# weikaolun/horovod-distributed-example

Measured on AMD Instinct MI355X. Metric: images/sec (whole node) + scaling efficiency, ResNet-50 bf16 at 1/2/4/8 MI355X, higher is better.
Workload: dtype bf16; 1 GPU; model=ResNet-50, global_batch=2048, per_gpu_batch=2048, image=224, parallelism=dp1, optimizer=mivod FusedSGD via DistributedOptimizer, compression=none, transport=local, hip_graph=False

## Files before the change

### csrc/kernels/mv_gemm.hip

```cpp
#include "mv_mfma.h"
#include "mv_gemm.h"

#include <cstdlib>

namespace mv {
namespace gemm {

constexpr int BK = 64;
constexpr int KC = BK / 8;

template <int BM, int BN, int WM, int WN, bool STATS>
__global__ __launch_bounds__(WM * WN * 64) void gemm_nt_kernel(
    const __bf16* __restrict__ A, const __bf16* __restrict__ B, __bf16* __restrict__ C,
    int64_t M, int N, int K, int ntn, const float* __restrict__ shift,
    float* __restrict__ partial) {
  constexpr int NT = WM * WN * 64;
  constexpr int A_CH = BM * KC / NT;
  constexpr int B_CH = BN * KC / NT;
  constexpr int WTM = BM / WM, WTN = BN / WN;
  constexpr int TM = WTM / 16, TN = WTN / 16;
  constexpr int STAGE = (BM + BN) * BK;
  static_assert(BM * KC % NT == 0 && BN * KC % NT == 0, "tile / thread mismatch");
  static_assert(WTM % 16 == 0 && WTN % 16 == 0, "wave tile");
  __shared__ __attribute__((aligned(16))) __bf16 smem[2 * STAGE];

  const int tid = threadIdx.x, lane = tid & 63, wid = tid >> 6;
  const int wm = wid / WN, wn = wid % WN;
  const int t = xcd_remap(blockIdx.x, gridDim.x);
  const int mt = t / ntn, nt = t - mt * ntn;
  const int64_t m0 = (int64_t)mt * BM;
  const int n0 = nt * BN;

  u32x4 ra[A_CH], rb[B_CH];
  auto gload = [&](int k0) {
#pragma unroll
    for (int i = 0; i < A_CH; ++i) {
      const int q = tid + i * NT, row = q / KC, ch = q % KC;
      int64_t gm = m0 + row;
      gm = gm < M ? gm : M - 1;
      ra[i] = *reinterpret_cast<const u32x4*>(A + gm * K + k0 + ch * 8);
    }
#pragma unroll
    for (int i = 0; i < B_CH; ++i) {
      const int q = tid + i * NT, row = q / KC, ch = q % KC;
      rb[i] = *reinterpret_cast<const u32x4*>(B + (int64_t)(n0 + row) * K + k0 + ch * 8);
    }
  };
  auto sstore = [&](int buf) {
    __bf16* As = smem + buf * STAGE;
    __bf16* Bs = As + BM * BK;
#pragma unroll
    for (int i = 0; i < A_CH; ++i) {
      const int q = tid + i * NT, row = q / KC, ch = q % KC;
      *reinterpret_cast<u32x4*>(As + swz64(row, ch)) = ra[i];
    }
#pragma unroll
    for (int i = 0; i < B_CH; ++i) {
      const int q = tid + i * NT, row = q / KC, ch = q % KC;
      *reinterpret_cast<u32x4*>(Bs + swz64(row, ch)) = rb[i];
    }
  };

  f32x4v acc[TN][TM];
#pragma unroll
  for (int a = 0; a < TN; ++a)
#pragma unroll
    for (int b = 0; b < TM; ++b) acc[a][b] = f32x4v{0.f, 0.f, 0.f, 0.f};

  const int KT = K / BK;
  gload(0);
  sstore(0);
  __syncthreads();
  for (int kt = 0; kt < KT; ++kt) {
    if (kt + 1 < KT) gload((kt + 1) * BK);
    const __bf16* As = smem + (kt & 1) * STAGE;
    const __bf16* Bs = As + BM * BK;
#pragma unroll
    for (int kk = 0; kk < BK / 32; ++kk) {
      const int ch = kk * 4 + (lane >> 4);
      bf16x8 wf[TN], af[TM];
#pragma unroll
      for (int a = 0; a < TN; ++a)
        wf[a] = *reinterpret_cast<const bf16x8*>(Bs + swz64(wn * WTN + a * 16 + (lane & 15), ch));
#pragma unroll
      for (int b = 0; b < TM; ++b)
        af[b] = *reinterpret_cast<const bf16x8*>(As + swz64(wm * WTM + b * 16 + (lane & 15), ch));
#pragma unroll
      for (int a = 0; a < TN; ++a)
#pragma unroll
        for (int b = 0; b < TM; ++b) acc[a][b] = mfma(wf[a], af[b], acc[a][b]);
    }
    if (kt + 1 < KT) sstore((kt + 1) & 1);
    __syncthreads();
  }

  const int g = lane >> 4, rl = lane & 15;
  float s1[TN][4], s2[TN][4];
#pragma unroll
  for (int a = 0; a < TN; ++a) {
    const int col = n0 + wn * WTN + a * 16 + 4 * g;
    float sh[4] = {0.f, 0.f, 0.f, 0.f};
    if (STATS && shift) {
#pragma unroll
      for (int r = 0; r < 4; ++r) sh[r] = shift[col + r];
    }
#pragma unroll
    for (int r = 0; r < 4; ++r) { s1[a][r] = 0.f; s2[a][r] = 0.f; }
#pragma unroll
    for (int b = 0; b < TM; ++b) {
      const int64_t row = m0 + wm * WTM + b * 16 + rl;
      if (row < M) {
        const f32x4v v = acc[a][b];
        u32x2 o = {cvt_pk_bf16(v[0], v[1]), cvt_pk_bf16(v[2], v[3])};
        *reinterpret_cast<u32x2*>(C + row * N + col) = o;
        if (STATS) {
#pragma unroll
          for (int r = 0; r < 4; ++r) {
            const float d = round_bf16(v[r]) - sh[r];
            s1[a][r] += d;
            s2[a][r] += d * d;
          }
        }
      }
    }
  }
  if (!STATS) return;
#pragma unroll
  for (int a = 0; a < TN; ++a)
#pragma unroll
    for (int r = 0; r < 4; ++r) {
#pragma unroll
      for (int o = 1; o < 16; o <<= 1) {
        s1[a][r] += __shfl_xor(s1[a][r], o, kWave);
        s2[a][r] += __shfl_xor(s2[a][r], o, kWave);
      }
    }
  float* red = reinterpret_cast<float*>(smem);
  if (rl == 0) {
#pragma unroll
    for (int a = 0; a < TN; ++a)
#pragma unroll
      for (int r = 0; r < 4; ++r) {
        const int c = wn * WTN + a * 16 + 4 * g + r;
        red[(0 * WM + wm) * BN + c] = s1[a][r];
        red[(1 * WM + wm) * BN + c] = s2[a][r];
      }
  }
  __syncthreads();
  for (int v = tid; v < 2 * BN; v += NT) {
    const int k = v / BN, c = v - k * BN;
    float s = 0.f;
#pragma unroll
    for (int w = 0; w < WM; ++w) s += red[(k * WM + w) * BN + c];
    partial[((int64_t)mt * 2 + k) * N + n0 + c] = s;
  }
}

struct BwdEpi {
  const __bf16* dy2;
  const uint8_t* mask;
  const __bf16* x;
  const float* mean;
  int ds, H, W;
  const float* sc;
  const float* bi;
  uint8_t* mo;
  const __bf16* a2;
  const float* badd;
  const float* rsc;
  const float* rbi;
  const __bf16* b2;
};

template <int NC>
__device__ __forceinline__ void ld_raw(const __bf16* p, uint32_t (&r)[NC / 2]) {
  if constexpr (NC == 4) {
    const u32x2 w = *reinterpret_cast<const u32x2*>(p);
    r[0] = w[0];
    r[1] = w[1];
  } else {
#pragma unroll
    for (int h = 0; h < NC / 8; ++h) {
      const u32x4 w = *reinterpret_cast<const u32x4*>(p + 8 * h);
#pragma unroll
      for (int j = 0; j < 4; ++j) r[4 * h + j] = w[j];
    }
  }
}

__device__ __forceinline__ float bf_lo(uint32_t w) { return __uint_as_float(w << 16); }
__device__ __forceinline__ float bf_hi(uint32_t w) { return __uint_as_float(w & 0xffff0000u); }

__device__ __forceinline__ int sw64(int row) {
  return (row & 2) | ((((row >> 2) ^ (row >> 4)) & 1) << 2);
}

__device__ __attribute__((aligned(16))) __bf16 g_zero_row[64];
__device__ __attribute__((aligned(16))) __bf16 g_store_scratch[512 * 16];
__device__ __attribute__((aligned(16))) uint8_t g_mask_scratch[512 * 4];

template <int K, int BN, int EPI>
constexpr int stream_wm() {
  if ((EPI == 4 || EPI == 6) && BN == 64) return K == 640 ? 4 : 2;
  return ((EPI == 2 || EPI == 3 || EPI == 5) && (BN == 256 || (K == 256 && BN == 128))) ||
                 ((EPI == 0 || EPI == 1 || EPI == 8) && K == 512)
             ? 2
             : 1;
}

template <int K, int BN, int EPI>
constexpr int stream_wn() {
  return (K == 256 && BN == 128 && (EPI == 2 || EPI == 3 || EPI == 5)) ||
                 ((EPI == 4 || EPI == 6) && BN == 64)
             ? 2
             : 4;
}
template <int K, int BN, int EPI>
constexpr int stream_nt() { return 64 * stream_wn<K, BN, EPI>() * stream_wm<K, BN, EPI>(); }

template <int K, int BN, int EPI, int BM = 64, int K1 = K>
__global__ __launch_bounds__((stream_nt<K, BN, EPI>())) void gemm_stream_kernel(
    const __bf16* __restrict__ A, const __bf16* __restrict__ B, __bf16* __restrict__ C,
    int64_t M, int N, int ntn, int64_t ntm, const float* __restrict__ shift,
    float* __restrict__ partial, BwdEpi be) {
  constexpr int WN = stream_wn<K, BN, EPI>();
  constexpr int NT = stream_nt<K, BN, EPI>();
  constexpr int WM = NT / (64 * WN);
  constexpr int KCH = K / 8;
  constexpr int A_CH = BM * KCH / NT;
  constexpr int W_CH = BN * KCH / NT;
  static_assert(A_CH * NT == BM * KCH && W_CH * NT == BN * KCH, "staging split");
  constexpr int WTN = BN / WN;
  constexpr int WTM = BM / WM;
  constexpr int TN = WTN / 16, TM = WTM / 16;
  constexpr int NC = 4 * TN;
  constexpr bool DUAL = EPI == 7;
  constexpr bool PF = (EPI == 2 || EPI == 3 || EPI == 5) && (BM == 32 || BN == 256);
  __shared__ __attribute__((aligned(16))) __bf16 smem[(BN + BM) * K * (DUAL ? 2 : 1)];
  __bf16* Ws = smem;
  __bf16* As = smem + BN * K;
  __bf16* Ws2 = smem + (BN + BM) * K;
  __bf16* As2 = Ws2 + BN * K;
  constexpr bool SW16 = K % 128 == 0 && K != 128;
  constexpr bool SW64 = K == 64;
  constexpr int LNC = NC == 4 ? 2 : (NC == 8 ? 3 : 4);
  auto swa = [](int row, int ch) {
    return row * K + ((ch ^ (SW16 ? (row & 15) : SW64 ? sw64(row) : (row & 7))) << 3);
  };
  auto sww = [](int row, int ch) {
    return row * K + ((ch ^ (SW16 ? ((row & 3) | (((row >> LNC) & 3) << 2))
                             : SW64 ? sw64(row) : (row & 7))) << 3);
  };

  const int tid = threadIdx.x, lane = tid & 63, wn = (tid >> 6) % WN;
  const int wm = (tid >> 6) / WN;
  const int g = lane >> 4, rl = lane & 15;
  const int t = xcd_remap(blockIdx.x, gridDim.x);
  const int nt = t % ntn;
  const int64_t stream = t / ntn, nstreams = gridDim.x / ntn;
  const int n0 = nt * BN;
  const int cbase = n0 + wn * WTN + NC * g;

#pragma unroll
  for (int i = 0; i < W_CH; ++i) {
    const int q = tid + i * NT, row = q / KCH, ch = q % KCH;
    *reinterpret_cast<u32x4*>(Ws + sww(row, ch)) =
        *reinterpret_cast<const u32x4*>(B + (int64_t)(n0 + row) * K + ch * 8);
    if constexpr (DUAL)
      *reinterpret_cast<u32x4*>(Ws2 + sww(row, ch)) =
          *reinterpret_cast<const u32x4*>(be.b2 + (int64_t)(n0 + row) * K + ch * 8);
  }
  u32x4 ra[A_CH], ra2[DUAL ? A_CH : 1];
  auto gload = [&](u32x4 (&ra)[A_CH], int64_t mt) {
    const int64_t m0 = mt * BM;
#pragma unroll
    for (int i = 0; i < A_CH; ++i) {
      const int q = tid + i * NT, row = q / KCH, ch = q % KCH;
      int64_t gm = m0 + row;
      gm = gm < M ? gm : M - 1;
      if constexpr (K1 == K) {
        ra[i] = *reinterpret_cast<const u32x4*>(A + gm * K + ch * 8);
        if constexpr (DUAL) ra2[i] = *reinterpret_cast<const u32x4*>(be.a2 + gm * K + ch * 8);
      } else {
        const __bf16* p = ch < K1 / 8 ? A + gm * K1 + ch * 8
                                      : be.a2 + gm * (K - K1) + (ch - K1 / 8) * 8;
        ra[i] = *reinterpret_cast<const u32x4*>(p);
      }
    }
  };
  float sh[NC], s1[NC], s2[NC];
  constexpr bool APPLY = EPI == 3 || EPI == 5 || EPI == 7;
  constexpr bool RAFF = EPI == 5 || EPI == 7;
  constexpr bool BADD = EPI == 4 || EPI == 6;
  float apl_sc[EPI >= 3 ? NC : 1], apl_bi[EPI >= 3 ? NC : 1], add[BADD ? NC : 1];
  float res_sc[RAFF ? NC : 1], res_bi[RAFF ? NC : 1];
  if constexpr (RAFF) {
#pragma unroll
    for (int j = 0; j < NC; ++j) {
      res_sc[j] = be.rsc[cbase + j];
      res_bi[j] = be.rbi[cbase + j];
    }
  }
  if constexpr (EPI == 4) {
#pragma unroll
    for (int j = 0; j < NC; ++j) {
      apl_sc[j] = be.sc[cbase + j];
      apl_bi[j] = be.bi[cbase + j];
    }
  }
  if constexpr (BADD) {
#pragma unroll
    for (int j = 0; j < NC; ++j) add[j] = be.badd[cbase + j];
  }
  if constexpr (APPLY) {
    static_assert(NC == 8 || NC == 16, "EPI 3 writes whole mask bytes");
#pragma unroll
    for (int j = 0; j < NC; ++j) {
      apl_sc[j] = be.sc[cbase + j];
      apl_bi[j] = be.bi[cbase + j];
    }
  }
#pragma unroll
  for (int j = 0; j < NC; ++j) {
    sh[j] = 0.f;
    if ((EPI == 1 || EPI == 8) && shift) sh[j] = shift[cbase + j];
    if (EPI == 2 || EPI == 4) sh[j] = be.mean[cbase + j];
    s1[j] = 0.f;
    s2[j] = 0.f;
  }
  struct Epi {
    uint32_t e2[EPI == 2 || APPLY ? TM : 1][NC / 2], ex[EPI == 2 || EPI == 4 ? TM : 1][NC / 2];
    uint32_t em[EPI == 2 ? TM : 1];
  };
  auto load_epi = [&](Epi& E, int64_t mt) {
    auto& e2 = E.e2;
    auto& ex = E.ex;
    auto& em = E.em;
    if constexpr (APPLY && !DUAL) {
#pragma unroll
      for (int b = 0; b < TM; ++b) {
        int64_t row = mt * BM + wm * WTM + b * 16 + rl;
        row = row < M ? row : M - 1;
        ld_raw<NC>(be.dy2 + row * N + cbase, e2[b]);
      }
    }
    if constexpr (EPI == 4) {
#pragma unroll
      for (int b = 0; b < TM; ++b) {
        int64_t row = mt * BM + wm * WTM + b * 16 + rl;
        row = row < M ? row : M - 1;
        ld_raw<NC>(be.x + row * N + cbase, ex[b]);
      }
    }
    if constexpr (EPI == 2) {
#pragma unroll
      for (int b = 0; b < TM; ++b) {
        int64_t row = mt * BM + wm * WTM + b * 16 + rl;
        row = row < M ? row : M - 1;
        int64_t r2 = row;
        bool has = be.dy2 != nullptr;
        if (be.ds > 1) {
          const uint32_t m = (uint32_t)row, hw = (uint32_t)(be.H * be.W);
          const uint32_t n = m / hw, rem = m - n * hw;
          const uint32_t h = rem / (uint32_t)be.W, w = rem - h * (uint32_t)be.W;
          const uint32_t hs = ((uint32_t)be.H + be.ds - 1) / be.ds;
          const uint32_t ws = ((uint32_t)be.W + be.ds - 1) / be.ds;
          has = has && h % be.ds == 0 && w % be.ds == 0;
          r2 = ((int64_t)n * hs + h / be.ds) * ws + w / be.ds;
        }
        ld_raw<NC>(has ? be.dy2 + r2 * N + cbase : g_zero_row, e2[b]);
        ld_raw<NC>(be.x ? be.x + row * N + cbase : g_zero_row, ex[b]);
        const uint8_t* mp = be.mask + row * (N / 8) + cbase / 8;
        if constexpr (NC == 4) em[b] = (uint32_t)mp[0] >> (cbase & 7);
        else if constexpr (NC == 8) em[b] = mp[0];
        else em[b] = *reinterpret_cast<const uint16_t*>(mp);
      }
    }
  };
  auto run_tile = [&](int64_t mt, Epi& E, Epi* En, u32x4 (&ra)[A_CH]) {
    auto& e2 = E.e2;
    auto& ex = E.ex;
    auto& em = E.em;
    (void)e2; (void)ex; (void)em;
    __syncthreads();
#pragma unroll
    for (int i = 0; i < A_CH; ++i) {
      const int q = tid + i * NT, row = q / KCH, ch = q % KCH;
      *reinterpret_cast<u32x4*>(As + swa(row, ch)) = ra[i];
      if constexpr (DUAL) *reinterpret_cast<u32x4*>(As2 + swa(row, ch)) = ra2[i];
    }
    __syncthreads();
    gload(ra, mt + nstreams < ntm ? mt + nstreams : mt);
    if constexpr (PF) {
      __builtin_amdgcn_sched_barrier(0);
      load_epi(*En, mt + nstreams < ntm ? mt + nstreams : mt);
      __builtin_amdgcn_sched_barrier(0);
    }
    f32x4v acc[TN][TM];
#pragma unroll
    for (int a = 0; a < TN; ++a)
#pragma unroll
      for (int b = 0; b < TM; ++b) acc[a][b] = f32x4v{0.f, 0.f, 0.f, 0.f};
    if constexpr (DUAL) {
      f32x4v acc2[TN][TM];
#pragma unroll
      for (int a = 0; a < TN; ++a)
#pragma unroll
        for (int b = 0; b < TM; ++b) acc2[a][b] = f32x4v{0.f, 0.f, 0.f, 0.f};
#pragma unroll
      for (int kk = 0; kk < K / 32; ++kk) {
        const int ch = kk * 4 + g;
        bf16x8 wf[TN], af[TM];
#pragma unroll
        for (int a = 0; a < TN; ++a)
          wf[a] = *reinterpret_cast<const bf16x8*>(
              Ws2 + sww(wn * WTN + NC * (rl >> 2) + 4 * a + (rl & 3), ch));
#pragma unroll
        for (int b = 0; b < TM; ++b)
          af[b] = *reinterpret_cast<const bf16x8*>(As2 + swa(wm * WTM + b * 16 + rl, ch));
#pragma unroll
        for (int a = 0; a < TN; ++a)
#pragma unroll
          for (int b = 0; b < TM; ++b) acc2[a][b] = mfma(wf[a], af[b], acc2[a][b]);
      }
#pragma unroll
      for (int b = 0; b < TM; ++b)
#pragma unroll
        for (int a = 0; a < TN; ++a) {
          e2[b][2 * a] = cvt_pk_bf16(acc2[a][b][0], acc2[a][b][1]);
          e2[b][2 * a + 1] = cvt_pk_bf16(acc2[a][b][2], acc2[a][b][3]);
        }
    }
#pragma unroll
    for (int kk = 0; kk < K / 32; ++kk) {
      const int ch = kk * 4 + g;
      bf16x8 wf[TN], af[TM];
#pragma unroll
      for (int a = 0; a < TN; ++a)
        wf[a] = *reinterpret_cast<const bf16x8*>(
            Ws + sww(wn * WTN + NC * (rl >> 2) + 4 * a + (rl & 3), ch));
#pragma unroll
      for (int b = 0; b < TM; ++b)
        af[b] = *reinterpret_cast<const bf16x8*>(As + swa(wm * WTM + b * 16 + rl, ch));
#pragma unroll
      for (int a = 0; a < TN; ++a)
#pragma unroll
        for (int b = 0; b < TM; ++b) acc[a][b] = mfma(wf[a], af[b], acc[a][b]);
    }
    const int64_t m0 = mt * BM;
#pragma unroll
    for (int b = 0; b < TM; ++b) {
      const int64_t row = m0 + wm * WTM + b * 16 + rl;
      const bool live = row < M;
      uint32_t pk[2 * TN];
#pragma unroll
      for (int a = 0; a < TN; ++a) {
        if constexpr (BADD) {
#pragma unroll
          for (int r = 0; r < 4; ++r) acc[a][b][r] += add[4 * a + r];
        }
        if constexpr (WM >= 2) {
          pk[2 * a] = cvt_pk_bf16_cc(acc[a][b][0], acc[a][b][1]);
          pk[2 * a + 1] = cvt_pk_bf16_cc(acc[a][b][2], acc[a][b][3]);
        } else {
          pk[2 * a] = cvt_pk_bf16(acc[a][b][0], acc[a][b][1]);
          pk[2 * a + 1] = cvt_pk_bf16(acc[a][b][2], acc[a][b][3]);
        }
      }
      float v[NC];
#pragma unroll
      for (int j = 0; j < NC / 2; ++j) {
        v[2 * j] = __uint_as_float(pk[j] << 16);
        v[2 * j + 1] = __uint_as_float(pk[j] & 0xffff0000u);
      }
      if (EPI == 1 || EPI == 8) {
#pragma unroll
        for (int j = 0; j < NC; ++j) {
          const float d = live ? v[j] - sh[j] : 0.f;
          s1[j] += d;
          s2[j] = __builtin_fmaf(d, d, s2[j]);
        }
      }
      if constexpr (EPI == 2) {
#pragma unroll
        for (int j = 0; j < NC / 2; ++j) {
          v[2 * j] += bf_lo(e2[b][j]);
          v[2 * j + 1] += bf_hi(e2[b][j]);
        }
        const float xk = be.x ? 1.f : 0.f;
#pragma unroll
        for (int j = 0; j < NC; ++j) {
          const float xv = (j & 1) ? bf_hi(ex[b][j >> 1]) : bf_lo(ex[b][j >> 1]);
          const float d = ((em[b] >> j) & 1u) ? v[j] : 0.f;
          v[j] = d;
          const float dl = live ? d : 0.f;
          s1[j] += dl;
          s2[j] += xk * dl * (xv - sh[j]);
        }
#pragma unroll
        for (int j = 0; j < NC / 2; ++j) pk[j] = cvt_pk_bf16(v[2 * j], v[2 * j + 1]);
      }
      if constexpr (EPI == 4) {
#pragma unroll
        for (int j = 0; j < NC; ++j) {
          const float xv = (j & 1) ? bf_hi(ex[b][j >> 1]) : bf_lo(ex[b][j >> 1]);
          const float d = __builtin_fmaf(xv, apl_sc[j], apl_bi[j]) > 0.f ? v[j] : 0.f;
          v[j] = d;
          const float dl = live ? d : 0.f;
          s1[j] += dl;
          s2[j] += dl * (xv - sh[j]);
        }
#pragma unroll
        for (int j = 0; j < NC / 2; ++j) pk[j] = cvt_pk_bf16(v[2 * j], v[2 * j + 1]);
      }
      if constexpr (APPLY) {
        uint32_t bits = 0;
#pragma unroll
        for (int j = 0; j < NC; ++j) {
          float r = (j & 1) ? bf_hi(e2[b][j >> 1]) : bf_lo(e2[b][j >> 1]);
          if constexpr (RAFF) r = round_bf16(__builtin_fmaf(r, res_sc[j], res_bi[j]));
          float a = __builtin_fmaf(v[j], apl_sc[j], apl_bi[j]);
          a += r;
          a = fmaxf(a, 0.f);
          v[j] = a;
          bits |= (a > 0.f ? 1u : 0u) << j;
        }
#pragma unroll
        for (int j = 0; j < NC / 2; ++j) pk[j] = cvt_pk_bf16(v[2 * j], v[2 * j + 1]);
        uint8_t* mp = live ? be.mo + row * (N / 8) + cbase / 8 : g_mask_scratch + 4 * threadIdx.x;
        if constexpr (NC == 8) *mp = (uint8_t)bits;
        else *reinterpret_cast<uint16_t*>(mp) = (uint16_t)bits;
      }
      if constexpr (EPI == 8) continue;
      __bf16* cp = live ? C + row * N + cbase : g_store_scratch + 16 * threadIdx.x;
      if constexpr (NC == 4) {
        *reinterpret_cast<u32x2*>(cp) = u32x2{pk[0], pk[1]};
      } else {
#pragma unroll
        for (int h = 0; h < NC / 8; ++h)
          *reinterpret_cast<u32x4*>(cp + 8 * h) =
              u32x4{pk[4 * h], pk[4 * h + 1], pk[4 * h + 2], pk[4 * h + 3]};
      }
    }
  };
  int64_t mt = stream;
  gload(ra, mt);
  if constexpr (!PF) {
    for (; mt < ntm; mt += nstreams) {
      Epi E;
      load_epi(E, mt);
      run_tile(mt, E, nullptr, ra);
    }
  } else {
    Epi E0, E1;
    load_epi(E0, mt);
    for (;;) {
      run_tile(mt, E0, &E1, ra);
      mt += nstreams;
      if (mt >= ntm) break;
      run_tile(mt, E1, &E0, ra);
      mt += nstreams;
      if (mt >= ntm) break;
    }
  }
  if (EPI == 0 || EPI == 6 || APPLY) return;
#pragma unroll
  for (int j = 0; j < NC; ++j) {
#pragma unroll
    for (int o = 1; o < 16; o <<= 1) {
      s1[j] += __shfl_xor(s1[j], o, kWave);
      s2[j] += __shfl_xor(s2[j], o, kWave);
    }
  }
  if (rl == 0 && stream < ntm) {
#pragma unroll
    for (int j = 0; j < NC; ++j) {
      partial[((stream * WM + wm) * 2 + 0) * N + cbase + j] = s1[j];
      partial[((stream * WM + wm) * 2 + 1) * N + cbase + j] = s2[j];
    }
  }
}

template <int BM, int BN, int WM, int WN>
static void launch(const __bf16* A, const __bf16* B, __bf16* C, int64_t M, int N, int K,
                   const float* shift, float* partial, hipStream_t st) {
  const int ntn = N / BN;
  const int64_t ntm = (M + BM - 1) / BM;
  const dim3 grid((unsigned)(ntm * ntn));
  if (partial)
    hipLaunchKernelGGL((gemm_nt_kernel<BM, BN, WM, WN, true>), grid, dim3(WM * WN * 64), 0, st, A,
                       B, C, M, N, K, ntn, shift, partial);
  else
    hipLaunchKernelGGL((gemm_nt_kernel<BM, BN, WM, WN, false>), grid, dim3(WM * WN * 64), 0, st,
                       A, B, C, M, N, K, ntn, shift, partial);
}

}
}

static bool stream_cfg(int K, int N, int* bn) {
  if (K == 64 || K == 128) { *bn = N % 256 == 0 ? 256 : (N % 128 == 0 ? 128 : 64); return true; }
  if (K == 256) { *bn = N % 128 == 0 ? 128 : 64; return true; }
  if (K == 512 && N % 256 != 0 && N % 64 == 0) { *bn = 64; return true; }
  return false;
}

template <int K, int EPI>
constexpr int stream_bm() { return (K == 256 && (EPI == 2 || EPI == 3 || EPI == 5)) ? 32 : 64; }

template <int K, int BN, int EPI>
static int64_t streams_for(int64_t M, int N) {
  constexpr int BMV = stream_bm<K, EPI>();
  static int per = [] {
    int v = 0;
    if (hipOccupancyMaxActiveBlocksPerMultiprocessor(
            &v, (const void*)&mv::gemm::gemm_stream_kernel<K, BN, EPI, BMV>,
            mv::gemm::stream_nt<K, BN, EPI>(), 0) != hipSuccess ||
        v < 1)
      v = 1;
    return v;
  }();
  const int ntn = N / BN;
  const int64_t ntm = (M + BMV - 1) / BMV;
  int64_t streams = (int64_t)mv::num_cus() * per / ntn;
  if (streams < 1) streams = 1;
  if (streams > ntm) streams = ntm;
  return streams;
}

template <int K, int BN>
static void launch_stream(const __bf16* a, const __bf16* b, __bf16* c, int64_t M, int N,
                          const float* shift, float* partial, const mv::gemm::BwdEpi* be,
                          hipStream_t st) {
  using namespace mv::gemm;
  const int ntn = N / BN;
  BwdEpi e{};
  if (be) {
    e = *be;
    constexpr int BMV = stream_bm<K, 2>();
    const int64_t ntm = (M + BMV - 1) / BMV;
    const dim3 grid((unsigned)(streams_for<K, BN, 2>(M, N) * ntn));
    hipLaunchKernelGGL((gemm_stream_kernel<K, BN, 2, BMV>), grid, dim3(stream_nt<K, BN, 2>()),
                       0, st, a, b, c, M, N,
                       ntn, ntm, shift, partial, e);
  } else if (partial) {
    const int64_t ntm = (M + 63) / 64;
    const dim3 grid((unsigned)(streams_for<K, BN, 1>(M, N) * ntn));
    static_assert(stream_wm<K, BN, 1>() == stream_wm<K, BN, 8>(), "one partial-row layout");
    if (c)
      hipLaunchKernelGGL((gemm_stream_kernel<K, BN, 1>), grid, dim3(stream_nt<K, BN, 1>()),
                         0, st, a, b, c, M, N, ntn, ntm, shift, partial, e);
    else
      hipLaunchKernelGGL((gemm_stream_kernel<K, BN, 8>), grid, dim3(stream_nt<K, BN, 8>()),
                         0, st, a, b, c, M, N, ntn, ntm, shift, partial, e);
  } else {
    const int64_t ntm = (M + 63) / 64;
    const dim3 grid((unsigned)(streams_for<K, BN, 0>(M, N) * ntn));
    hipLaunchKernelGGL((gemm_stream_kernel<K, BN, 0>), grid, dim3(stream_nt<K, BN, 0>()), 0,
                       st, a, b, c, M, N, ntn, ntm, shift, partial, e);
  }
}

template <int K, int BN>
static void launch_apply(const __bf16* a, const __bf16* b, __bf16* y, int64_t M, int N,
                         const mv::gemm::BwdEpi& e, hipStream_t st) {
  using namespace mv::gemm;
  if constexpr (BN >= 128) {
    const int ntn = N / BN;
    const int64_t ntm = (M + 63) / 64;
    if (e.b2) {
      if constexpr (K == 64) {
        const dim3 grid((unsigned)(streams_for<K, BN, 7>(M, N) * ntn));
        hipLaunchKernelGGL((gemm_stream_kernel<K, BN, 7>), grid, dim3(256), 0, st, a, b, y, M, N,
                           ntn, ntm, nullptr, nullptr, e);
      }
    } else if (e.rsc) {
      constexpr int BMV = stream_bm<K, 5>();
      const dim3 grid((unsigned)(streams_for<K, BN, 5>(M, N) * ntn));
      hipLaunchKernelGGL((gemm_stream_kernel<K, BN, 5, BMV>), grid, dim3(stream_nt<K, BN, 5>()), 0, st, a, b, y, M,
                         N, ntn, (M + BMV - 1) / BMV, nullptr, nullptr, e);
    } else {
      constexpr int BMV = stream_bm<K, 3>();
      const dim3 grid((unsigned)(streams_for<K, BN, 3>(M, N) * ntn));
      hipLaunchKernelGGL((gemm_stream_kernel<K, BN, 3, BMV>), grid, dim3(stream_nt<K, BN, 3>()), 0, st, a, b, y, M,
                         N, ntn, (M + BMV - 1) / BMV, nullptr, nullptr, e);
    }
  }
}

template <int K, int K1, int EPI = 4>
static bool launch_fold_dx(const __bf16* a, const __bf16* b, __bf16* d, int64_t M, int N,
                           const mv::gemm::BwdEpi& e, float* partial, int64_t* P, hipStream_t st) {
  using namespace mv::gemm;
  constexpr int BN = 64;
  static int per = [] {
    int v = 0;
    if (hipOccupancyMaxActiveBlocksPerMultiprocessor(
            &v, (const void*)&gemm_stream_kernel<K, BN, EPI, 64, K1>, stream_nt<K, BN, EPI>(),
            0) != hipSuccess || v < 1)
      v = 1;
    return v;
  }();
  const int ntn = N / BN;
  const int64_t ntm = (M + 63) / 64;
  int64_t streams = (int64_t)mv::num_cus() * per / ntn;
  if (streams < 1) streams = 1;
  if (streams > ntm) streams = ntm;
  *P = streams * stream_wm<K, BN, EPI>();
  if (EPI == 4 ? !partial : !a) return true;
  hipLaunchKernelGGL((gemm_stream_kernel<K, BN, EPI, 64, K1>), dim3((unsigned)(streams * ntn)),
                     dim3(stream_nt<K, BN, EPI>()), 0, st, a, b, d, M, N, ntn, ntm, nullptr,
                     partial, e);
  return true;
}

#define MV_STREAM_CASES(X) \
  X(64, 256) X(64, 128) X(64, 64) X(128, 256) X(128, 128) X(128, 64) X(256, 128) X(256, 64)

static bool gemm256_on() { return true; }

static bool g256_first(int64_t M, int N, int K) {
  return gemm256_on() && K == 256 && N % 256 == 0 && N >= 1024 && N <= 8192 &&
         mv_gemm256_supported(M, N, K);
}

int64_t mv_gemm_partials(int64_t M, int N, int K) {
  int bn;
  if (g256_first(M, N, K)) return mv_gemm256_partials(M, N);
  if (stream_cfg(K, N, &bn)) {
#define MV_P(KK, BB) \
    if (K == KK && bn == BB) return streams_for<KK, BB, 1>(M, N) * mv::gemm::stream_wm<KK, BB, 1>();
    MV_STREAM_CASES(MV_P)
    MV_P(512, 64)
#undef MV_P
  }
  if (gemm256_on() && mv_gemm256_supported(M, N, K)) return mv_gemm256_partials(M, N);
  const int bm = N % 128 == 0 ? 128 : 256;
  return (M + bm - 1) / bm;
}

void mv_gemm_nt(const void* A, const void* B, void* C, int64_t M, int N, int K,
                const float* shift, float* partial, hipStream_t st) {
  using namespace mv::gemm;
  const __bf16* a = (const __bf16*)A;
  const __bf16* b = (const __bf16*)B;
  __bf16* c = (__bf16*)C;
  int bn;
  if (g256_first(M, N, K) && mv_gemm256_nt(A, B, C, M, N, K, shift, partial, st)) return;
  if (stream_cfg(K, N, &bn)) {
#define MV_L(KK, BB) \
    if (K == KK && bn == BB) { launch_stream<KK, BB>(a, b, c, M, N, shift, partial, nullptr, st); return; }
    MV_STREAM_CASES(MV_L)
    MV_L(512, 64)
#undef MV_L
  }
  if (gemm256_on() && mv_gemm256_nt(A, B, C, M, N, K, shift, partial, st)) return;
  if (N % 256 == 0)
    launch<128, 256, 2, 2>(a, b, c, M, N, K, shift, partial, st);
  else if (N % 128 == 0)
    launch<128, 128, 2, 2>(a, b, c, M, N, K, shift, partial, st);
  else
    launch<256, 64, 4, 1>(a, b, c, M, N, K, shift, partial, st);
}

static bool bwd_cfg(int K, int N, int req, int* bn) {
  if (K != 64 && K != 128 && K != 256) return false;
  int b = req > 0 ? req : (K == 256 ? 128 : 256);
  if (K == 256 && b > 128) b = 128;
  while (b > 64 && N % b) b >>= 1;
  if (b != 64 && b != 128 && b != 256) return false;
  if (N % b) return false;
  *bn = b;
  return true;
}

int64_t mv_gemm_bwd_partials(int64_t M, int N, int K, int req_bn) {
  int bn;
  if (!bwd_cfg(K, N, req_bn, &bn)) return -1;
#define MV_PB(KK, BB) \
  if (K == KK && bn == BB) return streams_for<KK, BB, 2>(M, N) * mv::gemm::stream_wm<KK, BB, 2>();
  MV_STREAM_CASES(MV_PB)
#undef MV_PB
  return -1;
}

bool mv_gemm_nt_bn_bwd(const void* A, const void* B, void* DZ, int64_t M, int N, int K,
                       const void* dy2, const void* mask, const void* x, const float* mean,
                       float* partial, int req_bn, hipStream_t st, int dy2_stride, int H, int W) {
  using namespace mv::gemm;
  int bn;
  if (!bwd_cfg(K, N, req_bn, &bn)) return false;
  BwdEpi e{(const __bf16*)dy2, (const uint8_t*)mask, (const __bf16*)x, mean,
           dy2_stride > 1 ? dy2_stride : 1, H, W};
  const __bf16* a = (const __bf16*)A;
  const __bf16* b = (const __bf16*)B;
  __bf16* c = (__bf16*)DZ;
#define MV_LB(KK, BB) \
  if (K == KK && bn == BB) { launch_stream<KK, BB>(a, b, c, M, N, nullptr, partial, &e, st); return true; }
  MV_STREAM_CASES(MV_LB)
#undef MV_LB
  return false;
}

bool mv_gemm_apply_supported(int N, int K) {
  int bn;
  return K % 64 == 0 && N % 64 == 0 && stream_cfg(K, N, &bn) && bn >= 128;
}

bool mv_gemm_nt_apply(const void* A, const void* B, void* Y, int64_t M, int N, int K,
                      const void* res, const float* scale, const float* bias, void* mask,
                      hipStream_t st, const float* rscale, const float* rbias) {
  using namespace mv::gemm;
  int bn;
  if (!mv_gemm_apply_supported(N, K) || !stream_cfg(K, N, &bn)) return false;
  BwdEpi e{};
  e.dy2 = (const __bf16*)res;
  e.ds = 1;
  e.sc = scale;
  e.bi = bias;
  e.mo = (uint8_t*)mask;
  e.rsc = rscale;
  e.rbi = rscale ? rbias : nullptr;
  const __bf16* a = (const __bf16*)A;
  const __bf16* b = (const __bf16*)B;
  __bf16* y = (__bf16*)Y;
#define MV_LA(KK, BB) \
  if (K == KK && bn == BB && BB >= 128) { launch_apply<KK, BB>(a, b, y, M, N, e, st); return true; }
  MV_STREAM_CASES(MV_LA)
#undef MV_LA
  return false;
}

static bool fold_dx_dispatch(int K1, int K2, const __bf16* a, const __bf16* b, __bf16* d,
                             int64_t M, int N, const mv::gemm::BwdEpi& e, float* partial,
                             int64_t* P, hipStream_t st) {
  if (N % 64 || N != K2) return false;
  if (K1 == 256 && K2 == 64) return launch_fold_dx<320, 256>(a, b, d, M, N, e, partial, P, st);
  if (K1 == 512 && K2 == 128) return launch_fold_dx<640, 512>(a, b, d, M, N, e, partial, P, st);
  return false;
}

static bool fold_dx_g256(int64_t M, int K1, int K2) {
  return gemm256_on() && K1 % 64 == 0 && mv_gemm256_supported(M, K2, K1 + K2) && 4 * K2 <= 8192;
}

int64_t mv_gemm_fold_dx_partials(int64_t M, int K1, int K2) {
  int64_t P = -1;
  mv::gemm::BwdEpi e{};
  if (!fold_dx_dispatch(K1, K2, nullptr, nullptr, nullptr, M, K2, e, nullptr, &P, nullptr))
    return fold_dx_g256(M, K1, K2) ? mv_gemm256_partials(M, K2) : -1;
  return P;
}

bool mv_gemm_fold_dx(const void* A1, const void* A2, const void* B, const float* badd,
                     void* D, int64_t M, int K1, int K2, const void* x, const float* mean,
                     const float* scale, const float* bias, float* partial, hipStream_t st) {
  mv::gemm::BwdEpi e{};
  e.x = (const __bf16*)x;
  e.mean = mean;
  e.sc = scale;
  e.bi = bias;
  e.a2 = (const __bf16*)A2;
  e.badd = badd;
  e.ds = 1;
  int64_t P = 0;
  if (fold_dx_dispatch(K1, K2, nullptr, nullptr, nullptr, M, K2, e, nullptr, &P, nullptr))
    return fold_dx_dispatch(K1, K2, (const __bf16*)A1, (const __bf16*)B, (__bf16*)D, M, K2, e,
                            partial, &P, st);
  return fold_dx_g256(M, K1, K2) &&
         mv_gemm256_dual(A1, A2, B, badd, D, M, K1, K2, K2, x, mean, scale, bias, partial, st);
}

bool mv_gemm_dual_supported(int K1, int K2) {
  return (K1 == 256 && K2 == 64) || (gemm256_on() && K1 % 64 == 0 && K2 % 256 == 0);
}

bool mv_gemm_dual_bias(const void* A1, const void* A2, const void* B, const float* badd, void* D,
                       int64_t M, int K1, int K2, hipStream_t st) {
  if (!mv_gemm_dual_supported(K1, K2)) return false;
  if (K2 % 256 == 0)
    return mv_gemm256_dual(A1, A2, B, badd, D, M, K1, K2, K2, nullptr, nullptr, nullptr, nullptr,
                           nullptr, st);
  mv::gemm::BwdEpi e{};
  e.a2 = (const __bf16*)A2;
  e.badd = badd;
  e.ds = 1;
  int64_t P = 0;
  return launch_fold_dx<320, 256, 6>((const __bf16*)A1, (const __bf16*)B, (__bf16*)D, M, K2, e,
                                     nullptr, &P, st);
}

bool mv_gemm_apply_dual_supported(int N, int K) {
  int bn;
  return K == 64 && mv_gemm_apply_supported(N, K) && stream_cfg(K, N, &bn) && bn >= 128;
}

bool mv_gemm_nt_apply_dual(const void* A, const void* B, const void* A2, const void* B2, void* Y,
                           int64_t M, int N, int K, const float* scale, const float* bias,
                           const float* rscale, const float* rbias, void* mask, hipStream_t st) {
  if (!mv_gemm_apply_dual_supported(N, K) || !rscale || !rbias) return false;
  using namespace mv::gemm;
  int bn;
  stream_cfg(K, N, &bn);
  BwdEpi e{};
  e.ds = 1;
  e.sc = scale;
  e.bi = bias;
  e.mo = (uint8_t*)mask;
  e.rsc = rscale;
  e.rbi = rbias;
  e.a2 = (const __bf16*)A2;
  e.b2 = (const __bf16*)B2;
  const __bf16* a = (const __bf16*)A;
  const __bf16* b = (const __bf16*)B;
  __bf16* y = (__bf16*)Y;
  (void)bn;
  launch_apply<64, 128>(a, b, y, M, N, e, st);
  return true;
}
```

Before: 19030 images/sec.

## Stage streamed GEMM A tiles through multi-slot LDS ring with buffer loads

Replaces the register-staged A-tile prefetch in the streaming GEMM kernel with an NS-deep LDS ring. Tiles are filled by direct buffer-to-LDS loads issued several tiles ahead, and ordering relies on vmcnt waits plus a raw barrier, with no per-tile double __syncthreads. The change also retunes per-variant tile height (BM), wave layout and stage counts, extends epilogue prefetch to EPI 4, and folds the launch code into a shared launch_variant helper. The goal is to hide global-load latency and cut register pressure and barriers. The cost is more LDS per block, which may lower occupancy, and fragile vmcnt accounting.

```diff
diff --git a/csrc/kernels/mv_gemm.hip b/csrc/kernels/mv_gemm.hip
--- a/csrc/kernels/mv_gemm.hip
+++ b/csrc/kernels/mv_gemm.hip
@@ -199,15 +199,45 @@
 __device__ __attribute__((aligned(16))) __bf16 g_store_scratch[512 * 16];
 __device__ __attribute__((aligned(16))) uint8_t g_mask_scratch[512 * 4];
 
+template <int W>
+__device__ __forceinline__ int stream_swz(int row, int ch) {
+  constexpr bool SW16 = W % 128 == 0 && W != 128, SW64 = W == 64;
+  return row * W + ((ch ^ (SW16 ? (row & 15) : SW64 ? sw64(row) : (row & 7))) << 3);
+}
+
+template <int W, int BM, int NT>
+__device__ __forceinline__ void stream_issue(const __bf16* src, int64_t M, int64_t mt,
+                                             int64_t ntm, __bf16* img, int tid, int wave) {
+  constexpr int KC = W / 8, CNT = BM * KC / NT;
+  static_assert(CNT * NT == BM * KC, "staging split");
+  const bool in = mt < ntm;
+  const int64_t m0 = in ? mt * BM : 0;
+  const int rows = in ? (int)(M - m0 < BM ? M - m0 : BM) : 0;
+  const __amdgpu_buffer_rsrc_t rs = buffer_rsrc(src + m0 * W, (uint32_t)(rows * W * 2));
+#pragma unroll
+  for (int i = 0; i < CNT; ++i) {
+    const int q = tid + i * NT, row = q / KC;
+    const int ch = (stream_swz<W>(row, q % KC) - row * W) >> 3;
+    const int r = row < rows ? row : rows - 1;
+    blds16(rs, (uint32_t)((r * W + ch * 8) * 2), img + (i * NT + wave * 64) * 8);
+  }
+}
+
+template <int K, int BN, int EPI>
+constexpr int stream_bm() {
+  if (K == 512 || K == 640) return 32;
+  if (K == 256 && BN == 64) return 32;
+  return 64;
+}
 template <int K, int BN, int EPI>
 constexpr int stream_wm() {
-  if ((EPI == 4 || EPI == 6) && BN == 64) return K == 640 ? 4 : 2;
-  return ((EPI == 2 || EPI == 3 || EPI == 5) && (BN == 256 || (K == 256 && BN == 128))) ||
-                 ((EPI == 0 || EPI == 1 || EPI == 8) && K == 512)
-             ? 2
-             : 1;
-}
-
+  constexpr bool EOP = EPI == 2 || EPI == 3 || EPI == 5;
+  if (EPI == 4 || EPI == 6) return K == 640 ? 2 : 4;
+  if (K == 256 && BN == 128 && EOP) return 4;
+  if (K == 128 && BN == 256) return 2;
+  if (K == 512) return 2;
+  return EOP && BN == 256 ? 2 : 1;
+}
 template <int K, int BN, int EPI>
 constexpr int stream_wn() {
   return (K == 256 && BN == 128 && (EPI == 2 || EPI == 3 || EPI == 5)) ||
@@ -217,8 +247,15 @@
 }
 template <int K, int BN, int EPI>
 constexpr int stream_nt() { return 64 * stream_wn<K, BN, EPI>() * stream_wm<K, BN, EPI>(); }
-
-template <int K, int BN, int EPI, int BM = 64, int K1 = K>
+template <int K, int BN, int EPI>
+constexpr int stream_ns() {
+  if (K == 640) return 2;
+  if (K == 128 && BN == 256) return 4;
+  return 3;
+}
+
+template <int K, int BN, int EPI, int K1 = K, int BM = stream_bm<K, BN, EPI>(),
+          int NS = stream_ns<K, BN, EPI>()>
 __global__ __launch_bounds__((stream_nt<K, BN, EPI>())) void gemm_stream_kernel(
     const __bf16* __restrict__ A, const __bf16* __restrict__ B, __bf16* __restrict__ C,
     int64_t M, int N, int ntn, int64_t ntm, const float* __restrict__ shift,
@@ -235,17 +272,22 @@
   constexpr int TN = WTN / 16, TM = WTM / 16;
   constexpr int NC = 4 * TN;
   constexpr bool DUAL = EPI == 7;
-  constexpr bool PF = (EPI == 2 || EPI == 3 || EPI == 5) && (BM == 32 || BN == 256);
-  __shared__ __attribute__((aligned(16))) __bf16 smem[(BN + BM) * K * (DUAL ? 2 : 1)];
+  constexpr bool PF = EPI == 2 || EPI == 3 || EPI == 4 || EPI == 5;
+  constexpr int SLOT = BM * K;
+  static_assert(NS >= 2, "ring: one slot read, at least one in flight");
+  static_assert((BN + NS * BM) * K * (DUAL ? 2 : 1) * 2 <= 160 * 1024, "LDS");
+  __shared__ __attribute__((aligned(16))) __bf16 smem[(BN + NS * BM) * K * (DUAL ? 2 : 1)];
   __bf16* Ws = smem;
-  __bf16* As = smem + BN * K;
-  __bf16* Ws2 = smem + (BN + BM) * K;
-  __bf16* As2 = Ws2 + BN * K;
+  __bf16* Ar = smem + BN * K;
+  __bf16* Ws2 = smem + (BN + NS * BM) * K;
+  __bf16* Ar2 = Ws2 + BN * K;
   constexpr bool SW16 = K % 128 == 0 && K != 128;
   constexpr bool SW64 = K == 64;
   constexpr int LNC = NC == 4 ? 2 : (NC == 8 ? 3 : 4);
   auto swa = [](int row, int ch) {
-    return row * K + ((ch ^ (SW16 ? (row & 15) : SW64 ? sw64(row) : (row & 7))) << 3);
+    if constexpr (K1 == K) return stream_swz<K>(row, ch);
+    else return ch < K1 / 8 ? stream_swz<K1>(row, ch)
+                            : BM * K1 + stream_swz<K - K1>(row, ch - K1 / 8);
   };
   auto sww = [](int row, int ch) {
     return row * K + ((ch ^ (SW16 ? ((row & 3) | (((row >> LNC) & 3) << 2))
@@ -270,22 +312,16 @@
       *reinterpret_cast<u32x4*>(Ws2 + sww(row, ch)) =
           *reinterpret_cast<const u32x4*>(be.b2 + (int64_t)(n0 + row) * K + ch * 8);
   }
-  u32x4 ra[A_CH], ra2[DUAL ? A_CH : 1];
-  auto gload = [&](u32x4 (&ra)[A_CH], int64_t mt) {
-    const int64_t m0 = mt * BM;
-#pragma unroll
-    for (int i = 0; i < A_CH; ++i) {
-      const int q = tid + i * NT, row = q / KCH, ch = q % KCH;
-      int64_t gm = m0 + row;
-      gm = gm < M ? gm : M - 1;
-      if constexpr (K1 == K) {
-        ra[i] = *reinterpret_cast<const u32x4*>(A + gm * K + ch * 8);
-        if constexpr (DUAL) ra2[i] = *reinterpret_cast<const u32x4*>(be.a2 + gm * K + ch * 8);
-      } else {
-        const __bf16* p = ch < K1 / 8 ? A + gm * K1 + ch * 8
-                                      : be.a2 + gm * (K - K1) + (ch - K1 / 8) * 8;
-        ra[i] = *reinterpret_cast<const u32x4*>(p);
-      }
+  __syncthreads();
+  const int wave = __builtin_amdgcn_readfirstlane(tid >> 6);
+  auto issue = [&](int64_t mt, int slot) {
+    __bf16* img = Ar + slot * SLOT;
+    if constexpr (K1 == K) {
+      stream_issue<K, BM, NT>(A, M, mt, ntm, img, tid, wave);
+      if constexpr (DUAL) stream_issue<K, BM, NT>(be.a2, M, mt, ntm, Ar2 + slot * SLOT, tid, wave);
+    } else {
+      stream_issue<K1, BM, NT>(A, M, mt, ntm, img, tid, wave);
+      stream_issue<K - K1, BM, NT>(be.a2, M, mt, ntm, img + BM * K1, tid, wave);
     }
   };
   float sh[NC], s1[NC], s2[NC];
@@ -377,75 +413,80 @@
       }
     }
   };
-  auto run_tile = [&](int64_t mt, Epi& E, Epi* En, u32x4 (&ra)[A_CH]) {
+  constexpr int LDN = NC == 4 ? 1 : NC / 8;
+  constexpr int L_E = (EPI == 2 ? TM * (2 * LDN + 1) : 0) + (EPI == 4 ? TM * LDN : 0) +
+                      (APPLY && !DUAL ? TM * LDN : 0);
+  static_assert(PF == (L_E > 0), "every variant with epilogue operands prefetches them");
+  constexpr int A_D = A_CH * (DUAL ? 2 : 1);
+  constexpr int S_T = (EPI == 8 ? 0 : TM * LDN) + (APPLY ? TM : 0);
+  constexpr int PER = A_D + L_E + S_T;
+  constexpr int W_RING = L_E + S_T + (NS - 2) * PER;
+  static_assert(W_RING <= 63, "vmcnt is a 6-bit field");
+  auto run_tile = [&](int64_t mt, Epi& E, Epi* En, int rs, int ws) {
     auto& e2 = E.e2;
     auto& ex = E.ex;
     auto& em = E.em;
     (void)e2; (void)ex; (void)em;
-    __syncthreads();
-#pragma unroll
-    for (int i = 0; i < A_CH; ++i) {
-      const int q = tid + i * NT, row = q / KCH, ch = q % KCH;
-      *reinterpret_cast<u32x4*>(As + swa(row, ch)) = ra[i];
-      if constexpr (DUAL) *reinterpret_cast<u32x4*>(As2 + swa(row, ch)) = ra2[i];
-    }
-    __syncthreads();
-    gload(ra, mt + nstreams < ntm ? mt + nstreams : mt);
+    const __bf16* As = Ar + rs * SLOT;
+    const __bf16* As2 = Ar2 + rs * SLOT;
+    (void)As2;
+    issue(mt + (NS - 1) * nstreams, ws);
+    __builtin_amdgcn_sched_barrier(0);
+    f32x4v acc[TN][TM];
+#pragma unroll
+    for (int a = 0; a < TN; ++a)
+#pragma unroll
+      for (int b = 0; b < TM; ++b) acc[a][b] = f32x4v{0.f, 0.f, 0.f, 0.f};
+    if constexpr (DUAL) {
+      f32x4v acc2[TN][TM];
+#pragma unroll
+      for (int a = 0; a < TN; ++a)
+#pragma unroll
+        for (int b = 0; b < TM; ++b) acc2[a][b] = f32x4v{0.f, 0.f, 0.f, 0.f};
+#pragma unroll
+      for (int kk = 0; kk < K / 32; ++kk) {
+        const int ch = kk * 4 + g;
+        bf16x8 wf[TN], af[TM];
+#pragma unroll
+        for (int a = 0; a < TN; ++a)
+          wf[a] = *reinterpret_cast<const bf16x8*>(
+              Ws2 + sww(wn * WTN + NC * (rl >> 2) + 4 * a + (rl & 3), ch));
+#pragma unroll
+        for (int b = 0; b < TM; ++b)
+          af[b] = *reinterpret_cast<const bf16x8*>(As2 + swa(wm * WTM + b * 16 + rl, ch));
+#pragma unroll
+        for (int a = 0; a < TN; ++a)
+#pragma unroll
+          for (int b = 0; b < TM; ++b) acc2[a][b] = mfma(wf[a], af[b], acc2[a][b]);
+      }
+#pragma unroll
+      for (int b = 0; b < TM; ++b)
+#pragma unroll
+        for (int a = 0; a < TN; ++a) {
+          e2[b][2 * a] = cvt_pk_bf16(acc2[a][b][0], acc2[a][b][1]);
+          e2[b][2 * a + 1] = cvt_pk_bf16(acc2[a][b][2], acc2[a][b][3]);
+        }
+    }
+#pragma unroll
+    for (int kk = 0; kk < K / 32; ++kk) {
+      const int ch = kk * 4 + g;
+      bf16x8 wf[TN], af[TM];
+#pragma unroll
+      for (int a = 0; a < TN; ++a)
+        wf[a] = *reinterpret_cast<const bf16x8*>(
+            Ws + sww(wn * WTN + NC * (rl >> 2) + 4 * a + (rl & 3), ch));
+#pragma unroll
+      for (int b = 0; b < TM; ++b)
+        af[b] = *reinterpret_cast<const bf16x8*>(As + swa(wm * WTM + b * 16 + rl, ch));
+#pragma unroll
+      for (int a = 0; a < TN; ++a)
+#pragma unroll
+        for (int b = 0; b < TM; ++b) acc[a][b] = mfma(wf[a], af[b], acc[a][b]);
+    }
     if constexpr (PF) {
       __builtin_amdgcn_sched_barrier(0);
       load_epi(*En, mt + nstreams < ntm ? mt + nstreams : mt);
       __builtin_amdgcn_sched_barrier(0);
-    }
-    f32x4v acc[TN][TM];
-#pragma unroll
-    for (int a = 0; a < TN; ++a)
-#pragma unroll
-      for (int b = 0; b < TM; ++b) acc[a][b] = f32x4v{0.f, 0.f, 0.f, 0.f};
-    if constexpr (DUAL) {
-      f32x4v acc2[TN][TM];
-#pragma unroll
-      for (int a = 0; a < TN; ++a)
-#pragma unroll
-        for (int b = 0; b < TM; ++b) acc2[a][b] = f32x4v{0.f, 0.f, 0.f, 0.f};
-#pragma unroll
-      for (int kk = 0; kk < K / 32; ++kk) {
-        const int ch = kk * 4 + g;
-        bf16x8 wf[TN], af[TM];
-#pragma unroll
-        for (int a = 0; a < TN; ++a)
-          wf[a] = *reinterpret_cast<const bf16x8*>(
-              Ws2 + sww(wn * WTN + NC * (rl >> 2) + 4 * a + (rl & 3), ch));
-#pragma unroll
-        for (int b = 0; b < TM; ++b)
-          af[b] = *reinterpret_cast<const bf16x8*>(As2 + swa(wm * WTM + b * 16 + rl, ch));
-#pragma unroll
-        for (int a = 0; a < TN; ++a)
-#pragma unroll
-          for (int b = 0; b < TM; ++b) acc2[a][b] = mfma(wf[a], af[b], acc2[a][b]);
-      }
-#pragma unroll
-      for (int b = 0; b < TM; ++b)
-#pragma unroll
-        for (int a = 0; a < TN; ++a) {
-          e2[b][2 * a] = cvt_pk_bf16(acc2[a][b][0], acc2[a][b][1]);
-          e2[b][2 * a + 1] = cvt_pk_bf16(acc2[a][b][2], acc2[a][b][3]);
-        }
-    }
-#pragma unroll
-    for (int kk = 0; kk < K / 32; ++kk) {
-      const int ch = kk * 4 + g;
-      bf16x8 wf[TN], af[TM];
-#pragma unroll
-      for (int a = 0; a < TN; ++a)
-        wf[a] = *reinterpret_cast<const bf16x8*>(
-            Ws + sww(wn * WTN + NC * (rl >> 2) + 4 * a + (rl & 3), ch));
-#pragma unroll
-      for (int b = 0; b < TM; ++b)
-        af[b] = *reinterpret_cast<const bf16x8*>(As + swa(wm * WTM + b * 16 + rl, ch));
-#pragma unroll
-      for (int a = 0; a < TN; ++a)
-#pragma unroll
-        for (int b = 0; b < TM; ++b) acc[a][b] = mfma(wf[a], af[b], acc[a][b]);
     }
     const int64_t m0 = mt * BM;
 #pragma unroll
@@ -542,27 +583,39 @@
               u32x4{pk[4 * h], pk[4 * h + 1], pk[4 * h + 2], pk[4 * h + 3]};
       }
     }
+    __builtin_amdgcn_sched_barrier(0);
+    wait_vm<W_RING>();
+    raw_barrier();
   };
   int64_t mt = stream;
-  gload(ra, mt);
+  Epi E0, E1;
+  (void)E1;
+#pragma unroll
+  for (int p = 0; p < NS - 1; ++p) issue(mt + p * nstreams, p);
+  __builtin_amdgcn_sched_barrier(0);
+  if constexpr (PF) load_epi(E0, mt);
+  __builtin_amdgcn_sched_barrier(0);
+  wait_vm<0>();
+  raw_barrier();
+  int rs = 0, ws = NS - 1;
+  auto step = [&]() {
+    mt += nstreams;
+    rs = rs == NS - 1 ? 0 : rs + 1;
+    ws = ws == NS - 1 ? 0 : ws + 1;
+  };
   if constexpr (!PF) {
-    for (; mt < ntm; mt += nstreams) {
-      Epi E;
-      load_epi(E, mt);
-      run_tile(mt, E, nullptr, ra);
-    }
+    for (; mt < ntm; step()) run_tile(mt, E0, nullptr, rs, ws);
   } else {
-    Epi E0, E1;
-    load_epi(E0, mt);
     for (;;) {
-      run_tile(mt, E0, &E1, ra);
-      mt += nstreams;
+      run_tile(mt, E0, &E1, rs, ws);
+      step();
       if (mt >= ntm) break;
-      run_tile(mt, E1, &E0, ra);
-      mt += nstreams;
+      run_tile(mt, E1, &E0, rs, ws);
+      step();
       if (mt >= ntm) break;
     }
   }
+  wait_vm<0>();
   if (EPI == 0 || EPI == 6 || APPLY) return;
 #pragma unroll
   for (int j = 0; j < NC; ++j) {
@@ -605,27 +658,36 @@
   return false;
 }
 
-template <int K, int EPI>
-constexpr int stream_bm() { return (K == 256 && (EPI == 2 || EPI == 3 || EPI == 5)) ? 32 : 64; }
-
-template <int K, int BN, int EPI>
+template <int K, int BN, int EPI, int K1 = K>
 static int64_t streams_for(int64_t M, int N) {
-  constexpr int BMV = stream_bm<K, EPI>();
+  constexpr int BM = mv::gemm::stream_bm<K, BN, EPI>();
   static int per = [] {
     int v = 0;
     if (hipOccupancyMaxActiveBlocksPerMultiprocessor(
-            &v, (const void*)&mv::gemm::gemm_stream_kernel<K, BN, EPI, BMV>,
+            &v, (const void*)&mv::gemm::gemm_stream_kernel<K, BN, EPI, K1>,
             mv::gemm::stream_nt<K, BN, EPI>(), 0) != hipSuccess ||
         v < 1)
       v = 1;
     return v;
   }();
   const int ntn = N / BN;
-  const int64_t ntm = (M + BMV - 1) / BMV;
+  const int64_t ntm = (M + BM - 1) / BM;
   int64_t streams = (int64_t)mv::num_cus() * per / ntn;
   if (streams < 1) streams = 1;
   if (streams > ntm) streams = ntm;
   return streams;
+}
+
+template <int K, int BN, int EPI, int K1 = K>
+static void launch_variant(const __bf16* a, const __bf16* b, __bf16* c, int64_t M, int N,
+                           const float* shift, float* partial, const mv::gemm::BwdEpi& e,
+                           int64_t streams, hipStream_t st) {
+  using namespace mv::gemm;
+  constexpr int BM = stream_bm<K, BN, EPI>();
+  const int ntn = N / BN;
+  hipLaunchKernelGGL((gemm_stream_kernel<K, BN, EPI, K1>), dim3((unsigned)(streams * ntn)),
+                     dim3(stream_nt<K, BN, EPI>()), 0, st, a, b, c, M, N, ntn,
+                     (M + BM - 1) / BM, shift, partial, e);
 }
 
 template <int K, int BN>
@@ -633,57 +695,32 @@
                           const float* shift, float* partial, const mv::gemm::BwdEpi* be,
                           hipStream_t st) {
   using namespace mv::gemm;
-  const int ntn = N / BN;
   BwdEpi e{};
   if (be) {
-    e = *be;
-    constexpr int BMV = stream_bm<K, 2>();
-    const int64_t ntm = (M + BMV - 1) / BMV;
-    const dim3 grid((unsigned)(streams_for<K, BN, 2>(M, N) * ntn));
-    hipLaunchKernelGGL((gemm_stream_kernel<K, BN, 2, BMV>), grid, dim3(stream_nt<K, BN, 2>()),
-                       0, st, a, b, c, M, N,
-                       ntn, ntm, shift, partial, e);
+    launch_variant<K, BN, 2>(a, b, c, M, N, shift, partial, *be, streams_for<K, BN, 2>(M, N), st);
   } else if (partial) {
-    const int64_t ntm = (M + 63) / 64;
-    const dim3 grid((unsigned)(streams_for<K, BN, 1>(M, N) * ntn));
-    static_assert(stream_wm<K, BN, 1>() == stream_wm<K, BN, 8>(), "one partial-row layout");
-    if (c)
-      hipLaunchKernelGGL((gemm_stream_kernel<K, BN, 1>), grid, dim3(stream_nt<K, BN, 1>()),
-                         0, st, a, b, c, M, N, ntn, ntm, shift, partial, e);
-    else
-      hipLaunchKernelGGL((gemm_stream_kernel<K, BN, 8>), grid, dim3(stream_nt<K, BN, 8>()),
-                         0, st, a, b, c, M, N, ntn, ntm, shift, partial, e);
+    const int64_t streams = streams_for<K, BN, 1>(M, N);
+    static_assert(stream_wm<K, BN, 1>() == stream_wm<K, BN, 8>() &&
+                      stream_bm<K, BN, 1>() == stream_bm<K, BN, 8>(),
+                  "one partial-row layout");
+    if (c) launch_variant<K, BN, 1>(a, b, c, M, N, shift, partial, e, streams, st);
+    else launch_variant<K, BN, 8>(a, b, c, M, N, shift, partial, e, streams, st);
   } else {
-    const int64_t ntm = (M + 63) / 64;
-    const dim3 grid((unsigned)(streams_for<K, BN, 0>(M, N) * ntn));
-    hipLaunchKernelGGL((gemm_stream_kernel<K, BN, 0>), grid, dim3(stream_nt<K, BN, 0>()), 0,
-                       st, a, b, c, M, N, ntn, ntm, shift, partial, e);
+    launch_variant<K, BN, 0>(a, b, c, M, N, shift, partial, e, streams_for<K, BN, 0>(M, N), st);
   }
 }
 
 template <int K, int BN>
 static void launch_apply(const __bf16* a, const __bf16* b, __bf16* y, int64_t M, int N,
                          const mv::gemm::BwdEpi& e, hipStream_t st) {
-  using namespace mv::gemm;
   if constexpr (BN >= 128) {
-    const int ntn = N / BN;
-    const int64_t ntm = (M + 63) / 64;
     if (e.b2) {
-      if constexpr (K == 64) {
-        const dim3 grid((unsigned)(streams_for<K, BN, 7>(M, N) * ntn));
-        hipLaunchKernelGGL((gemm_stream_kernel<K, BN, 7>), grid, dim3(256), 0, st, a, b, y, M, N,
-                           ntn, ntm, nullptr, nullptr, e);
-      }
+      if constexpr (K == 64)
+        launch_variant<K, BN, 7>(a, b, y, M, N, nullptr, nullptr, e, streams_for<K, BN, 7>(M, N), st);
     } else if (e.rsc) {
-      constexpr int BMV = stream_bm<K, 5>();
-      const dim3 grid((unsigned)(streams_for<K, BN, 5>(M, N) * ntn));
-      hipLaunchKernelGGL((gemm_stream_kernel<K, BN, 5, BMV>), grid, dim3(stream_nt<K, BN, 5>()), 0, st, a, b, y, M,
-                         N, ntn, (M + BMV - 1) / BMV, nullptr, nullptr, e);
+      launch_variant<K, BN, 5>(a, b, y, M, N, nullptr, nullptr, e, streams_for<K, BN, 5>(M, N), st);
     } else {
-      constexpr int BMV = stream_bm<K, 3>();
-      const dim3 grid((unsigned)(streams_for<K, BN, 3>(M, N) * ntn));
-      hipLaunchKernelGGL((gemm_stream_kernel<K, BN, 3, BMV>), grid, dim3(stream_nt<K, BN, 3>()), 0, st, a, b, y, M,
-                         N, ntn, (M + BMV - 1) / BMV, nullptr, nullptr, e);
+      launch_variant<K, BN, 3>(a, b, y, M, N, nullptr, nullptr, e, streams_for<K, BN, 3>(M, N), st);
     }
   }
 }
@@ -691,26 +728,11 @@
 template <int K, int K1, int EPI = 4>
 static bool launch_fold_dx(const __bf16* a, const __bf16* b, __bf16* d, int64_t M, int N,
                            const mv::gemm::BwdEpi& e, float* partial, int64_t* P, hipStream_t st) {
-  using namespace mv::gemm;
   constexpr int BN = 64;
-  static int per = [] {
-    int v = 0;
-    if (hipOccupancyMaxActiveBlocksPerMultiprocessor(
-            &v, (const void*)&gemm_stream_kernel<K, BN, EPI, 64, K1>, stream_nt<K, BN, EPI>(),
-            0) != hipSuccess || v < 1)
-      v = 1;
-    return v;
-  }();
-  const int ntn = N / BN;
-  const int64_t ntm = (M + 63) / 64;
-  int64_t streams = (int64_t)mv::num_cus() * per / ntn;
-  if (streams < 1) streams = 1;
-  if (streams > ntm) streams = ntm;
-  *P = streams * stream_wm<K, BN, EPI>();
+  const int64_t streams = streams_for<K, BN, EPI, K1>(M, N);
+  *P = streams * mv::gemm::stream_wm<K, BN, EPI>();
   if (EPI == 4 ? !partial : !a) return true;
-  hipLaunchKernelGGL((gemm_stream_kernel<K, BN, EPI, 64, K1>), dim3((unsigned)(streams * ntn)),
-                     dim3(stream_nt<K, BN, EPI>()), 0, st, a, b, d, M, N, ntn, ntm, nullptr,
-                     partial, e);
+  launch_variant<K, BN, EPI, K1>(a, b, d, M, N, nullptr, partial, e, streams, st);
   return true;
 }
 
```

Result: no change. 19050 images/sec (median of 6 runs) (+0.1%).
